# KRLGroup/gym-ma-survival-2d

Hardware: NVIDIA B200
Metric: agent_steps_per_sec (higher is better)
Workload: dtype f32

## Files before the change

### gym-ma-survival-2d_b200/csrc/msv_env.cuh

```cuda
#pragma once
#include "msv_device.cuh"
#include "msv_types.cuh"
#include "msv_launch.h"

enum { F_CX, F_CY, F_A, F_VX, F_VY, F_W, F_C0X, F_C0Y, F_A0, F_ALPHA0, F_SLEEP,
       F_FAT0, F_FAT1, F_FAT2, F_FAT3, F_FLAGS, F_QS, F_QC, F_COUNT };
enum { G_X, G_Y, G_HX, G_HY, G_AX, G_AY, G_ROT, G_F0, G_F1, G_F2, G_F3, G_COUNT };
enum { K_META, K_SEQ, K_MTYPE, K_LNX, K_LNY, K_LPX, K_LPY, K_NI, K_TI, K_NM, K_TM, K_COUNT };
enum { KS_NX = K_SEQ, KS_NY = K_MTYPE, KS_PX = K_LNX, KS_PY = K_LNY, KS_RBX = K_LPX, KS_RBY = K_LPY };

#define FL_ALIVE 1
#define FL_AWAKE 2
#define FL_ISLAND 4
#define FL_MOVED 8

#define KIND_NONE 0
#define KIND_AGENT 1
#define KIND_BOX 2
#define KIND_ITEM 3
#define KIND_HEAL 4
#define KIND_WALL 5

#define STREAM_SHUFFLE 0
#define STREAM_BOX 1
// ... 13 lines not shown
  int sid;
  int b;
  int flags;
  Manifold m;
  float ni, ti;
  f2 normal, rA, rB;
  float normalMass, tangentMass;
};

struct BodyS { f2 c; float a; f2 v; float w; float invM, invI; };

extern __shared__ float msv_sm[];


#ifndef MSV_INLINE_MASK
#define MSV_INLINE_MASK 0
#endif
#ifndef MSV_TOI_COOP
#define MSV_TOI_COOP 0
#endif
#ifndef MSV_FIXPOINT
#define MSV_FIXPOINT 1
#endif
#if (MSV_INLINE_MASK >> 0) & 1
#define COLD0 __device__ __forceinline__
#else
#define COLD0 __device__ __noinline__
#endif
#if (MSV_INLINE_MASK >> 1) & 1
#define COLD1 __device__ __forceinline__
#else
#define COLD1 __device__ __noinline__
#endif
#if (MSV_INLINE_MASK >> 2) & 1
#define COLD2 __device__ __forceinline__
#else
#define COLD2 __device__ __noinline__
#endif
#if (MSV_INLINE_MASK >> 3) & 1
#define COLD3 __device__ __forceinline__
#else
#define COLD3 __device__ __noinline__
#endif
#if (MSV_INLINE_MASK >> 4) & 1
#define COLD4 __device__ __forceinline__
#else
#define COLD4 __device__ __noinline__
#endif

__device__ __noinline__ double2 philox_uniform2_of(const DevConst& C, uint32_t genv, uint32_t episode, uint32_t step, uint32_t stream, uint32_t blk) {
  uint32_t o[4];
  philox4x32(genv, episode, step, (stream << 16) | blk, C.seed_lo, C.seed_hi, o);
  return make_double2(((double)(o[0] >> 5) * 67108864.0 + (double)(o[1] >> 6)) / 9007199254740992.0,
                      ((double)(o[2] >> 5) * 67108864.0 + (double)(o[3] >> 6)) / 9007199254740992.0);
}

__device__ __noinline__ void draw_reset(const DevConst& C, uint32_t genv, uint32_t episode, float* rec) {
  const int n = C.grid_n;
  unsigned char perm[64];
  for (int k = 0; k < n; ++k) perm[k] = (unsigned char)k;
  double2 up = make_double2(0.0, 0.0);
  for (int i = n - 1; i >= 1; --i) {
    const uint32_t kd = (uint32_t)(n - 1 - i);
    if (!(kd & 1u)) up = philox_uniform2_of(C, genv, episode, 0u, STREAM_SHUFFLE, kd >> 1);
    const double u = (kd & 1u) ? up.y : up.x;
    const int j = (int)(u * (i + 1));
    const unsigned char t = perm[i]; perm[i] = perm[j]; perm[j] = t;
  }
  int top = n;
  for (int b = 0; b < C.B0; ++b) {
    float hx = C.box_h, hy = C.box_h;
    if (C.box_randomized) {
// ... 72 lines not shown
  DEV void gsync() const { __syncwarp(gmask); }
  template <class V> DEV V bc(V v) const { return __shfl_sync(gmask, v, 0, G); }
  template <class V> DEV V from(V v, int j) const { return __shfl_sync(gmask, v, j, G); }
  DEV unsigned or32(unsigned v) const {
#pragma unroll
    for (int o = 1; o < G; o <<= 1) v |= __shfl_xor_sync(gmask, v, o, G);
    return v;
  }
  DEV unsigned long long or64(unsigned long long v) const {
#pragma unroll
    for (int o = 1; o < G; o <<= 1) v |= __shfl_xor_sync(gmask, v, o, G);
    return v;
  }
  DEV void share_counts() { int c = bc(nb | (ni << 8) | (nh << 16)); nb = c & 255; ni = (c >> 8) & 255; nh = (c >> 16) & 255; }
  DEV void share_bits() {
#pragma unroll
    for (int w = 0; w < PW; ++w) { ex[w] = bc(ex[w]); tc[w] = bc(tc[w]); en[w] = bc(en[w]); }
  }
  DEV void merge_bits() {
#pragma unroll
    for (int w = 0; w < PW; ++w) { ex[w] = or64(ex[w] & own[w]); tc[w] = or64(tc[w] & own[w]); en[w] = or64(en[w] & own[w]); }
  }

  DEV void take(const Env& o) {
    nb = o.nb; ni = o.ni; nh = o.nh; ntc = o.ntc;
#pragma unroll
    for (int w = 0; w < PW; ++w) { ex[w] = o.ex[w]; tc[w] = o.tc[w]; en[w] = o.en[w]; }
  }
#define MSV_COLD(call) do { Env c_(*this); c_.call; take(c_); } while (0)
#ifndef MSV_INLINE_MASK
#define MSV_INLINE_MASK 0
#endif
#define MSV_COLDK(k, call) do { if ((MSV_INLINE_MASK >> (k)) & 1) { call; } else { Env c_(*this); c_.call; take(c_); } } while (0)

  DEV float& AG(int f, int i) { return msv_sm[sb + (CHK_IDX(f, F_COUNT) * AC + CHK_IDX(i, AC))]; }
  DEV int& AGF(int i) { return reinterpret_cast<int*>(msv_sm)[sb + (F_FLAGS * AC + CHK_IDX(i, AC))]; }
  DEV float& BX(int f, int k) { return msv_sm[sb + (W_BOX + CHK_IDX(f, G_COUNT) * BC + CHK_IDX(k, BC))]; }
  DEV int& BXROT(int k) { return reinterpret_cast<int*>(msv_sm)[sb + (W_BOX + G_ROT * BC + CHK_IDX(k, BC))]; }
  DEV float& KF(int f, int k) { return msv_sm[sb + (W_TC + CHK_IDX(f, K_COUNT) * MAXC + CHK_IDX(k, MAXC))]; }
  DEV int& KI(int f, int k) { return reinterpret_cast<int*>(msv_sm)[sb + (W_TC + CHK_IDX(f, K_COUNT) * MAXC + CHK_IDX(k, MAXC))]; }
  DEV int& NTC() { return reinterpret_cast<int*>(msv_sm)[sb + (W_MISC + 0)]; }
  DEV float& ITP(int c, int k) { return msv_sm[sb + (W_ITEM + CHK_IDX(c, 2) * BC + CHK_IDX(k, BC))]; }
  DEV float& HLP(int c, int k) { return msv_sm[sb + (W_HEAL + CHK_IDX(c, 2) * HC + CHK_IDX(k, HC))]; }
  DEV int& LI(int k) { return reinterpret_cast<int*>(msv_sm)[sb + (W_LEAD + CHK_IDX(k, L_COUNT))]; }
  DEV unsigned& LU(int k) { return reinterpret_cast<unsigned*>(msv_sm)[sb + (W_LEAD + CHK_IDX(k, L_COUNT))]; }
  DEV float& LF(int k) { return msv_sm[sb + (W_LEAD + CHK_IDX(k, L_COUNT))]; }
  DEV float& TOIA(int i, int k) { return msv_sm[sb + (W_TOI + CHK_IDX(i, AC) * (BC + 4) + CHK_IDX(k, BC + 4))]; }
  DEV int& OVF() { return reinterpret_cast<int*>(msv_sm)[sb + (W_MISC + 1)]; }
  DEV bool alive(int i) { return AGF(i) & FL_ALIVE; }
  DEV bool awake(int i) { return AGF(i) & FL_AWAKE; }
  DEV f2 apos(int i) { return mk2(AG(F_CX, i), AG(F_CY, i)); }
  DEV static int meta_pack(int p, int a, int sid, int b) { return p | ((a + 1) << 8) | ((sid < 0 ? 0 : sid) << 12) | (b << 16); }
  DEV static void meta_unpack(int m, int& p, int& a, int& sid, int& b) { p = m & 255; a = ((m >> 8) & 15) - 1; sid = (m >> 12) & 15; b = (m >> 16) & 15; }

  DEV static bool bit(const unsigned long long* m, int p) {
    unsigned long long w = m[0];
// ... 194 lines not shown
  }
  DEV void box_change_health(int k, int delta, int cz) {
    int4 b1 = S.box1[k * N + e];
    if (!(b1.y & 1)) return;
    if (b1.w != MSV_CAUSE_NONE && cz != b1.w) return;
    b1.x += delta; b1.z = cz;
    S.box1[k * N + e] = b1;
  }
  DEV int inv_n(int i) { return LI(L_INV + (i)) & 7; }
  DEV int inv_kind(int i, int s) { return (LI(L_INV + (i)) >> (4 + 2 * s)) & 3; }
  DEV void inv_push(int i, int kind, float4 payload) {
    int n = inv_n(i);
    LI(L_INV + (i)) = (LI(L_INV + (i)) & ~(3 << (4 + 2 * n)) & ~7) | (kind << (4 + 2 * n)) | (n + 1);
    if (kind == MSV_ITEM_BOX) S.ainv[(i * 4 + n) * N + e] = payload;
  }
  DEV int inv_pop(int i, float4& payload) {
    int n = inv_n(i) - 1;
    int kind = inv_kind(i, n);
    if (kind == MSV_ITEM_BOX) payload = S.ainv[(i * 4 + n) * N + e];
    LI(L_INV + (i)) = (LI(L_INV + (i)) & ~7) | n;
    return kind;
  }

  COLD3 void remove_box(int k) {
    for (int i = 0; i < C.A; ++i) {
      int p = p_ab(i, k);
      if (bit(ex, p) && bit(tc, p)) wake(i);
      for (int q = k; q + 1 < nb; ++q) {
        int pd = p_ab(i, q), ps = p_ab(i, q + 1);
        if (bit(ex, ps)) { setb(ex, pd); S.pseq[pd * N + e] = S.pseq[ps * N + e]; S.pimp[pd * N + e] = S.pimp[ps * N + e]; } else clrb(ex, pd);
        if (bit(tc, ps)) setb(tc, pd); else clrb(tc, pd);
        if (bit(en, ps)) setb(en, pd); else clrb(en, pd);
      }
      int pl = p_ab(i, nb - 1);
      clrb(ex, pl); clrb(tc, pl); clrb(en, pl);
    }
    for (int q = k; q + 1 < nb; ++q) {
      S.box0[q * N + e] = S.box0[(q + 1) * N + e];
      S.box1[q * N + e] = S.box1[(q + 1) * N + e];
      S.boxseq[q * N + e] = S.boxseq[(q + 1) * N + e];
      BX(G_X, q) = BX(G_X, q + 1); BX(G_Y, q) = BX(G_Y, q + 1); BX(G_HX, q) = BX(G_HX, q + 1);
      BX(G_HY, q) = BX(G_HY, q + 1); BX(G_AX, q) = BX(G_AX, q + 1); BX(G_AY, q) = BX(G_AY, q + 1);
      BXROT(q) = BXROT(q + 1);
      BX(G_F0, q) = BX(G_F0, q + 1); BX(G_F1, q) = BX(G_F1, q + 1); BX(G_F2, q) = BX(G_F2, q + 1); BX(G_F3, q) = BX(G_F3, q + 1);
    }
    nb--;
  }
// ... 34 lines not shown
  DEV void candidates_of(int j, unsigned long long* cand, bool only_moved = false) {
    const int fj_ = AGF(j);
    if (!(fj_ & FL_ALIVE)) return;
    const bool mj = !only_moved || (fj_ & FL_MOVED);
    float fj[4]; agent_fat(j, fj);
    for (int i = 0; i < j; ++i) {
      const int fi_ = AGF(i);
      if (!(fi_ & FL_ALIVE)) continue;
      if (!mj && !(fi_ & FL_MOVED)) continue;
      int p = p_aa(i, j);
      if (bit(ex, p)) continue;
      float fi[4]; agent_fat(i, fi);
      if (aabb_overlap(fi, fj)) setb(cand, p);
    }
    if (!mj) return;
    for (int k = 0; k < BC + 4; ++k) {
      if (k < BC && k >= nb) continue;
      int p = k < BC ? p_ab(j, k) : p_aw(j, k - BC);
      if (bit(ex, p)) continue;
      float fs[4]; static_fat(k, fs);
      if (aabb_overlap(fj, fs)) setb(cand, p);
    }
  }
  COLD2 void number_candidates(unsigned long long* cand) {
    for (;;) {
      int best = -1; unsigned bestKey = 0xFFFFFFFFu;
      for (int w = 0; w < PW; ++w) {
        unsigned long long m = cand[w];
        while (m) {
          int p = w * 64 + __ffsll((long long)m) - 1; m &= m - 1;
          int a, sid, b; decode(p, a, sid, b);
          int s1 = a >= 0 ? agent_seq(a) : static_seq(sid), s2 = agent_seq(b);
          int lo = s1 < s2 ? s1 : s2, hi = s1 < s2 ? s2 : s1;
          unsigned key = ((unsigned)lo << 16) | (unsigned)hi;
          if (key < bestKey) { bestKey = key; best = p; }
        }
      }
      if (best < 0) break;
      clrb(cand, best);
      setb(ex, best); setb(en, best); clrb(tc, best);
      S.pseq[best * N + e] = (uint32_t)(++LI(L_CONTACTSEQ));
      S.pimp[best * N + e] = make_float2(0.0f, 0.0f);
    }
  }
  DEV void find_new_contacts(bool only_moved = false) {
    unsigned long long cand[PW];
#pragma unroll
    for (int w = 0; w < PW; ++w) cand[w] = 0ull;
    for (int j = g; j < C.A; j += G) candidates_of(j, cand, only_moved);
    bool any = false;
#pragma unroll
    for (int w = 0; w < PW; ++w) { cand[w] = or64(cand[w]); any |= cand[w] != 0ull; }
    if (any) {
      if (lead) {
        int nset = 0;
#pragma unroll
        for (int w = 0; w < PW; ++w) nset += __popcll(cand[w]);
        if (nset == 1) {
          int p = 0;
#pragma unroll
          for (int w = 0; w < PW; ++w) if (cand[w]) p = w * 64 + __ffsll((long long)cand[w]) - 1;
          setb(ex, p); setb(en, p); clrb(tc, p);
          S.pseq[p * N + e] = (uint32_t)(++LI(L_CONTACTSEQ));
          S.pimp[p * N + e] = make_float2(0.0f, 0.0f);
        } else { RARE_BEGIN(); unsigned long long cc[PW]; for (int w = 0; w < PW; ++w) cc[w] = cand[w]; MSV_COLDK(2, number_candidates(cc)); RARE_END(6); }
      }
      share_bits();
    }
  }
  DEV void find_new_contacts_of(int b) {
    unsigned long long cand[PW];
#pragma unroll
    for (int w = 0; w < PW; ++w) cand[w] = 0ull;
    candidates_of(b, cand);
    float fb[4]; agent_fat(b, fb);
    for (int j = b + 1; j < C.A; ++j) {
      if (!(AGF(j) & FL_ALIVE)) continue;
      const int p = p_aa(b, j);
      if (bit(ex, p)) continue;
      float fj[4]; agent_fat(j, fj);
      if (aabb_overlap(fb, fj)) setb(cand, p);
    }
    bool any = false;
#pragma unroll
    for (int w = 0; w < PW; ++w) any |= cand[w] != 0ull;
    if (any) number_candidates(cand);
  }

// ... 246 lines not shown
    float r = C.agent_r;
    float c0x = AG(F_C0X, i), c0y = AG(F_C0Y, i), cx = AG(F_CX, i), cy = AG(F_CY, i);
    float a1[4] = {c0x - r, c0y - r, c0x + r, c0y + r};
    float a2[4] = {cx - r, cy - r, cx + r, cy + r};
    float ab[4] = {fmin_(a1[0], a2[0]), fmin_(a1[1], a2[1]), fmax_(a1[2], a2[2]), fmax_(a1[3], a2[3])};
    float f0 = AG(F_FAT0, i), f1 = AG(F_FAT1, i), f2_ = AG(F_FAT2, i), f3 = AG(F_FAT3, i);
    if (f0 <= ab[0] && f1 <= ab[1] && ab[2] <= f2_ && ab[3] <= f3) return;
    float n0 = ab[0] - B2_AABB_EXT, n1 = ab[1] - B2_AABB_EXT, n2 = ab[2] + B2_AABB_EXT, n3 = ab[3] + B2_AABB_EXT;
    float dx = B2_AABB_MULT * (cx - c0x), dy = B2_AABB_MULT * (cy - c0y);
    if (dx < 0.0f) n0 += dx; else n2 += dx;
    if (dy < 0.0f) n1 += dy; else n3 += dy;
    AG(F_FAT0, i) = n0; AG(F_FAT1, i) = n1; AG(F_FAT2, i) = n2; AG(F_FAT3, i) = n3;
    AGF(i) |= FL_MOVED;
  }

  template <int NRr>
  DEV void island_single(int i, int cnt, unsigned long long ord, float h, float dtRatio) {
    f2 cB = apos(i);
    AG(F_C0X, i) = cB.x; AG(F_C0Y, i) = cB.y; AG(F_A0, i) = AG(F_A, i);
    f2 vB = mk2(C.damp * AG(F_VX, i), C.damp * AG(F_VY, i)); float wB = AG(F_W, i) * C.damp;
    f2 nrm[NRr], pp[NRr];
    bool ok = true;
    if (cnt > 0) {
      f2 rB[NRr]; float nm[NRr], tm[NRr], ni_[NRr], ti_[NRr]; int pr[NRr];
#pragma unroll (NRr <= NR ? NRr : 1)
      for (int k = 0; k < NRr; ++k) {
        if (k < cnt) {
          int s = (int)((ord >> (5 * k)) & 31ull);
          int a_, sid, b_; meta_unpack(KI(K_META, s), pr[k], a_, sid, b_);
          ni_[k] = dtRatio * KF(K_NI, s); ti_[k] = dtRatio * KF(K_TI, s);
          init_velocity_static(sid, mk2(KF(K_LNX, s), KF(K_LNY, s)), mk2(KF(K_LPX, s), KF(K_LPY, s)), cB,
                               nrm[k], pp[k], rB[k], nm[k], tm[k]);
        }
      }
#pragma unroll (NRr <= NR ? NRr : 1)
      for (int k = 0; k < NRr; ++k) if (k < cnt) warm_start_static(nrm[k], rB[k], ni_[k], ti_[k], vB, wB);
      for (int it = 0; it < 10; ++it) {
        const f2 v_in = vB; const float w_in = wB; bool changed = false;
#pragma unroll (NRr <= NR ? NRr : 1)
        for (int k = 0; k < NRr; ++k) if (k < cnt) {
          const float n0 = ni_[k], t0 = ti_[k];
          solve_velocity_static(nrm[k], rB[k], nm[k], tm[k], ni_[k], ti_[k], vB, wB);
          changed |= (__float_as_uint(ni_[k]) != __float_as_uint(n0)) | (__float_as_uint(ti_[k]) != __float_as_uint(t0));
        }
        if (MSV_FIXPOINT && !changed && __float_as_uint(vB.x) == __float_as_uint(v_in.x) && __float_as_uint(vB.y) == __float_as_uint(v_in.y) &&
            __float_as_uint(wB) == __float_as_uint(w_in)) break;
      }
#pragma unroll (NRr <= NR ? NRr : 1)
      for (int k = 0; k < NRr; ++k) if (k < cnt) S.pimp[pr[k] * N + e] = make_float2(ni_[k], ti_[k]);
    }
    AG(F_VX, i) = vB.x; AG(F_VY, i) = vB.y; AG(F_W, i) = wB;
    integrate_position(i, h);
    if (cnt > 0) {
      ok = false;
      cB = apos(i);
      for (int it = 0; it < 10 && !ok; ++it) {
        float minSep = 0.0f;
#pragma unroll (NRr <= NR ? NRr : 1)
        for (int k = 0; k < NRr; ++k) if (k < cnt) minSep = fmin_(minSep, solve_position_static(nrm[k], pp[k], cB, false));
        ok = minSep >= -3.0f * B2_LINEAR_SLOP;
      }
      AG(F_CX, i) = cB.x; AG(F_CY, i) = cB.y;
    }
    {
      const float linTol = B2_LIN_SLEEP_TOL * B2_LIN_SLEEP_TOL, angTol = B2_ANG_SLEEP_TOL * B2_ANG_SLEEP_TOL;
      float w = AG(F_W, i); f2 v = mk2(AG(F_VX, i), AG(F_VY, i));
      float st;
      if (w * w > angTol || vdot(v, v) > linTol) st = 0.0f; else st = AG(F_SLEEP, i) + h;
      AG(F_SLEEP, i) = st;
      if (ok && st >= B2_TIME_TO_SLEEP) sleep_body(i);
    }
    synchronize_fixtures(i);
  }
  DEV void solve_single(int i, float h, float dtRatio) {
    int f = AGF(i);
    if (!(f & FL_ALIVE) || !(f & FL_AWAKE)) return;
    AGF(i) = f | FL_ISLAND;
    unsigned long long ord = 0ull; int cnt = 0; unsigned taken = 0;
    for (;;) {
      int best = -1, bestSeq = -1;
      for (int k = 0; k < ntc; ++k) {
        if ((taken >> k) & 1u) continue;
        int p, a_, sid, b_; meta_unpack(KI(K_META, k), p, a_, sid, b_);
        if (b_ != i || a_ >= 0) continue;
        if (!bit(en, p) || !bit(tc, p)) continue;
        int sq = KI(K_SEQ, k);
        if (sq > bestSeq) { bestSeq = sq; best = k; }
      }
      if (best < 0) break;
      taken |= 1u << best;
      ord |= (unsigned long long)best << (5 * cnt); cnt++;
    }
    SUB_BEGIN();
    if (cnt <= NR) island_single<NR>(i, cnt, ord, h, dtRatio);
    else island_single<BC + 4>(i, cnt, ord, h, dtRatio);
    SUBMAX(cnt <= NR ? 6 : 7, cnt);
  }

  struct Ord { unsigned long long lo, hi; };
  DEV static int ord_get(const Ord& o, int k) { return k < 12 ? (int)((o.lo >> (5 * k)) & 31ull) : (int)((o.hi >> (5 * (k - 12))) & 31ull); }
  DEV static void ord_put(Ord& o, int k, int v) { if (k < 12) o.lo |= (unsigned long long)v << (5 * k); else o.hi |= (unsigned long long)v << (5 * (k - 12)); }
  static constexpr int NP = 3;
  DEV void island_pair(unsigned inisl, int nc, const Ord& ord, float h, float dtRatio) {
    const int X = __ffs((int)inisl) - 1, Y = 31 - __clz((int)inisl);
    f2 cX = apos(X), cY = apos(Y);
    f2 vX = mk2(AG(F_VX, X), AG(F_VY, X)), vY = mk2(AG(F_VX, Y), AG(F_VY, Y));
    float wX = AG(F_W, X), wY = AG(F_W, Y), aX = AG(F_A, X), aY = AG(F_A, Y);
    const float mI = C.inv_mass, iI = C.inv_I;
    int ty[NP], pr[NP];
    f2 nrm[NP], px[NP], rB[NP]; float nm[NP], tm[NP], ni_[NP], ti_[NP];
#pragma unroll
    for (int k = 0; k < NP; ++k) {
      ty[k] = 0; pr[k] = 0; nrm[k] = mk2(0.f, 0.f); px[k] = nrm[k]; rB[k] = nrm[k]; nm[k] = tm[k] = ni_[k] = ti_[k] = 0.0f;
      if (k >= nc) continue;
      const int s = ord_get(ord, k);
      int a_, sid, b_; meta_unpack(KI(K_META, s), pr[k], a_, sid, b_);
      ni_[k] = dtRatio * KF(K_NI, s); ti_[k] = dtRatio * KF(K_TI, s);
      if (a_ >= 0) {
// ... 92 lines not shown
          cY = vadd(cY, vmul(mI, Pv)); aY += iI * vcross(rB_, Pv);
        }
        minSep = fmin_(minSep, separation);
      }
      ok = minSep >= -3.0f * B2_LINEAR_SLOP;
    }
    AG(F_CX, X) = cX.x; AG(F_CY, X) = cX.y; AG(F_A, X) = aX; AG(F_CX, Y) = cY.x; AG(F_CY, Y) = cY.y; AG(F_A, Y) = aY;
    {
      const float linTol = B2_LIN_SLEEP_TOL * B2_LIN_SLEEP_TOL, angTol = B2_ANG_SLEEP_TOL * B2_ANG_SLEEP_TOL;
      bool can_sleep = ok;
#pragma unroll
      for (int q = 0; q < 2; ++q) {
        const int i = q == 0 ? X : Y;
        float w = AG(F_W, i); f2 v = mk2(AG(F_VX, i), AG(F_VY, i));
        float st;
        if (w * w > angTol || vdot(v, v) > linTol) st = 0.0f; else st = AG(F_SLEEP, i) + h;
        AG(F_SLEEP, i) = st;
        if (!(st >= B2_TIME_TO_SLEEP)) can_sleep = false;
      }
      if (can_sleep) { sleep_body(X); sleep_body(Y); }
    }
    synchronize_fixtures(X); synchronize_fixtures(Y);
  }
  COLD0 void solve_island(int seed, float h, float dtRatio) {
    SUB_BEGIN();
    Ord ord; ord.lo = 0ull; ord.hi = 0ull;
    int nc = 0; unsigned taken = 0, inisl = 1u << seed;
    {
      unsigned stack = (unsigned)seed; int sc = 1;
      AGF(seed) |= FL_ISLAND;
      while (sc > 0) {
        --sc;
        const int bI = (int)((stack >> (4 * sc)) & 15u);
        wake(bI);
        for (;;) {
          int best = -1, bestSeq = -1, bestMeta = 0;
          for (int k = 0; k < ntc; ++k) {
            if ((taken >> k) & 1u) continue;
            const int meta = KI(K_META, k);
            int p, a_, sid, b_; meta_unpack(meta, p, a_, sid, b_);
            if (a_ != bI && b_ != bI) continue;
            if (!bit(en, p) || !bit(tc, p)) continue;
            const int sq = KI(K_SEQ, k);
            if (sq > bestSeq) { bestSeq = sq; best = k; bestMeta = meta; }
          }
          if (best < 0) break;
          taken |= 1u << best;
// ... 192 lines not shown
    }
    gsync();
  }
  __device__ __forceinline__ void solve_find_new() {
    unsigned mv = 0;
    for (int i = g; i < C.A; i += G) if (AGF(i) & FL_MOVED) mv = 1u;
    if (or32(mv)) find_new_contacts(true);
  }

  DEV void advance(int i, float alpha) {
    float a0 = AG(F_ALPHA0, i);
    float beta = (alpha - a0) / (1.0f - a0);
    AG(F_C0X, i) += beta * (AG(F_CX, i) - AG(F_C0X, i));
    AG(F_C0Y, i) += beta * (AG(F_CY, i) - AG(F_C0Y, i));
    AG(F_A0, i) += beta * (AG(F_A, i) - AG(F_A0, i));
    AG(F_ALPHA0, i) = alpha;
    AG(F_CX, i) = AG(F_C0X, i); AG(F_CY, i) = AG(F_C0Y, i); AG(F_A, i) = AG(F_A0, i);
  }

  static constexpr int SNAPW = F_COUNT + 6 * PW + 1;
  static constexpr int TOI_ISL = 8;
  static_assert(SNAPW <= K_COUNT * (MAXC - TOI_ISL), "snapshot does not fit the scratch slots");
  DEV unsigned& SNAP(int q) { CHK((unsigned)q < (unsigned)SNAPW); return reinterpret_cast<unsigned*>(msv_sm)[sb + (W_TC + (q / (MAXC - TOI_ISL)) * MAXC + TOI_ISL + q % (MAXC - TOI_ISL))]; }
  COLD1 int toi_event(int minP, float minAlpha, float dt, int prevP) {
    SUB_BEGIN();
    int a, sid, b; decode(minP, a, sid, b);
    const float bk0 = AG(F_C0X, b), bk1 = AG(F_C0Y, b), bk2 = AG(F_CX, b), bk3 = AG(F_CY, b), bk4 = AG(F_A0, b), bk5 = AG(F_A, b), bk6 = AG(F_ALPHA0, b);
    advance(b, minAlpha);
    int nisl = 0;
    auto isl_add = [&](int sid_, const Manifold& m) {
      SBox bx = static_box(sid_);
      const f2 normal = qmul(bx.qs, bx.qc, m.localNormal), planePoint = sb_mul(bx, m.localPoint);
      KF(KS_NX, nisl) = normal.x; KF(KS_NY, nisl) = normal.y; KF(KS_PX, nisl) = planePoint.x; KF(KS_PY, nisl) = planePoint.y;
      nisl++;
    };
    {
      Manifold m_min; unsigned wk = 0;
      bool touching = contact_update(minP, a, sid, b, false, wk, &m_min);
      wake_all(wk);
      if (!touching) {
        clrb(en, minP);
        AG(F_C0X, b) = bk0; AG(F_C0Y, b) = bk1; AG(F_CX, b) = bk2; AG(F_CY, b) = bk3;
        AG(F_A0, b) = bk4; AG(F_A, b) = bk5; AG(F_ALPHA0, b) = bk6;
        return 0;
      }
      wake(b);
      isl_add(sid, m_min);
// ... 154 lines not shown
        gsync();
        cvalid |= need;
        while (need) {
          const int k = __ffs((int)need) - 1; need &= need - 1u;
          consider(k < BC ? p_ab(i, k) : p_aw(i, k - BC), TOIA(i, k));
        }
      }
#pragma unroll
      for (int o = 1; o < G; o <<= 1) {
        float oa = __shfl_xor_sync(gmask, minAlpha, o, G);
        int op = __shfl_xor_sync(gmask, minP, o, G), os = __shfl_xor_sync(gmask, minSeq, o, G);
        if (op >= 0 && (oa < minAlpha || (oa == minAlpha && os > minSeq))) { minAlpha = oa; minP = op; minSeq = os; }
      }
      if (minP < 0 || 1.0f - 10.0f * B2_EPS < minAlpha) break;
      int ea, ek, eb; decode(minP, ea, ek, eb);
      const bool mine = eb == g;
      if (mine) cvalid &= ~(1u << ek);
      gsync();
      int r = 0;
      TOIPROF(long long tpe = clock64();)
      if (lead) {
        RARE_BEGIN();
        if ((MSV_INLINE_MASK >> 1) & 1) r = toi_event(minP, minAlpha, dt, prevP);
        else { Env c_(*this); r = c_.toi_event(minP, minAlpha, dt, prevP); take(c_); }
        if (r & 1) prevP = minP;
        RARE_END(1);
      }
      gsync();
      r = bc(r);
      TOIPROF(tp_ev += clock64() - tpe; if (r & 1) tp_ran++; else tp_not++; if (r & 2) tp_same++;)
      share_bits();
      if (mine) {
        const unsigned long long c4 = (evcnt >> (4 * ek)) & 15ull;
        if (c4 < 15ull) evcnt += 1ull << (4 * ek);
      }
      if (!(r & 1)) continue;
      if (mine) {
        if (r & 2) {
          const unsigned long long c4 = (evcnt >> (4 * ek)) & 15ull;
          if (c4 <= (unsigned long long)C.toi_max_count) evcnt = (evcnt & ~(15ull << (4 * ek))) | ((unsigned long long)(C.toi_max_count + 1) << (4 * ek));
        } else cvalid = 0u;
      }
    }
    gsync();
    TOIPROF(if (lead) { unsigned long long tot = (unsigned long long)(clock64() - tp0); unsigned long long old = atomicMax(&g_toi[0], tot);
      if (tot > old) { g_toi[1] = tp_it; g_toi[2] = tp_ran; g_toi[3] = tp_not; g_toi[4] = tp_same; g_toi[5] = (unsigned long long)tp_ev; g_toi[6] = tot - (unsigned long long)tp_ev; g_toi[7] = tp_calls; g_toi[8] = (unsigned long long)e; } })
  }
// ... 5 lines not shown
      if (real) {
        const uint8_t* a = actions + ((size_t)e * C.A + i) * 6;
        a0 = min((int)a[0], 2); a1 = min((int)a[1], 2); a2 = min((int)a[2], 2);
        flags |= (a[3] ? 1u : 0u) << i | (a[4] ? 1u : 0u) << (8 + i) | (a[5] ? 1u : 0u) << (16 + i);
      }
      if (!alive(i)) continue;
      float s, c; rot_set(AG(F_A, i), s, c);
      AG(F_QS, i) = s; AG(F_QC, i) = c;
      float par = C.imp_par[a0], nor = C.imp_nor[a1];
      float ix = c * par + (-s) * nor, iy = s * par + c * nor;
      wake(i);
      AG(F_VX, i) += C.inv_mass * ix; AG(F_VY, i) += C.inv_mass * iy;
      AG(F_W, i) += C.inv_I * C.imp_ang[a2];
    }
    return or32(flags);
  }
  DEV void pre_use_give(unsigned act) {
    LI(L_USEHEAL) = 0; LI(L_USEBOX) = 0; LI(L_NEWBOX) = 0;
    bool any = LI(L_NP) > 0;
#pragma unroll
    for (int i = 0; i < AC; ++i) if (i < C.A && (((act >> (8 + i)) | (act >> (16 + i))) & 1u) && (LI(L_INV + (i)) & 7) != 0 && alive(i)) any = true;
    if (any) { RARE_BEGIN(); MSV_COLDK(3, pre_use_give_body(act)); RARE_END(5); }
  }
  COLD3 void pre_use_give_body(unsigned act) {
    for (int q = 0; q < LI(L_NP); ++q) {
      float4 p0 = S.pend0[q * N + e];
      add_item(p0.x, p0.y, p0.z, p0.w, S.pend1[q * N + e]);
    }
    LI(L_NP) = 0;
#pragma unroll
    for (int i = 0; i < AC; ++i) {
      if (i >= C.A || !alive(i) || !((act >> (8 + i)) & 1u) || inv_n(i) == 0) continue;
      float4 pl; int kind = inv_pop(i, pl);
      if (kind == MSV_ITEM_HEAL) { LI(L_USEHEAL)++; agent_change_health(i, C.healing, MSV_CAUSE_NONE); }
      else {
        LI(L_USEBOX)++;
        if (nb >= BC) { LI(L_OVERFLOW)++; continue; }
        float L = C.box_item_offset;
        float qs = AG(F_QS, i), qc = AG(F_QC, i);
        f2 off = mk2(qc * L + (-qs) * 0.0f, qs * L + qc * 0.0f);
        float x = AG(F_CX, i) + off.x, y = AG(F_CY, i) + off.y;
        int reh = __float_as_int(pl.w) & 1;
        const float4 nb0 = make_float4(x, y, pl.x, pl.y);
        const int4 nb1 = make_int4(0, reh << 1, MSV_CAUSE_NONE, C.box_ownership ? __float_as_int(pl.z) : MSV_CAUSE_NONE);
        S.box0[nb * N + e] = nb0; S.box1[nb * N + e] = nb1;
        S.boxseq[nb * N + e] = LI(L_BODYSEQ)++;
        put_box(nb, nb0, nb1);
// ... 53 lines not shown
        }
#pragma unroll
        for (int j = 0; j < G; ++j) res[s * G + j] = from(r, j);
      }
      if (lead) {
#pragma unroll
        for (int i = 0; i < AC; ++i) {
          if (!((raymask >> i) & 1u)) continue;
          int kind = res[i] & 255, tidx = (res[i] >> 8) & 255;
          if (kind == KIND_NONE) continue;
          int cz = C.teams ? MSV_CAUSE_TEAM0 + team_of(i) : i;
          if (kind == KIND_AGENT) agent_change_health(tidx, -C.melee_damage, cz);
          else if (kind == KIND_BOX) box_change_health(tidx, -C.melee_damage, cz);
          if (C.melee_cooldown >= 0) LI(L_COOLDOWN + (i)) = C.melee_cooldown;
        }
      }
    }
    if (lead && C.melee_cooldown >= 0) {
#pragma unroll
      for (int i = 0; i < AC; ++i) if (LI(L_COOLDOWN + (i)) > 0) LI(L_COOLDOWN + (i))--;
    }
  }

  __device__ __noinline__ double philox_uniform(uint32_t step, uint32_t stream, uint32_t k) {
    uint32_t o[4];
    philox4x32(C.env_offset + (uint32_t)e, (uint32_t)LI(L_EPISODE), step, (stream << 16) | (k >> 1), C.seed_lo, C.seed_hi, o);
    uint32_t a = o[(k & 1) * 2], b = o[(k & 1) * 2 + 1];
    return ((double)(a >> 5) * 67108864.0 + (double)(b >> 6)) / 9007199254740992.0;
  }

  DEV bool in_cone(f2 pl) {
    bool inside = true;
#pragma unroll
    for (int v = 0; v < 4; ++v) {
      float d = vdot(mk2(C.cone_n[v][0], C.cone_n[v][1]), vsub(pl, mk2(C.cone_v[v][0], C.cone_v[v][1])));
      if (d > 0.0f) inside = false;
    }
    return inside;
  }
  DEV f2 target_pos(int t) {
    if (t < AC) return apos(t);
    t -= AC;
    if (t < BC) return mk2(BX(G_X, t), BX(G_Y, t));
    t -= BC;
    if (t < BC) return mk2(ITP(0, t), ITP(1, t));
    t -= BC;
    return mk2(HLP(0, t), HLP(1, t));
// ... 63 lines not shown

  __device__ __forceinline__ void post_step_boxes() {
    int4 b1s[BC];
#pragma unroll
    for (int j = 0; j < BC; ++j) if (j < nb) b1s[j] = S.box1[j * N + e];
    const int nb0 = nb; int removed = 0;
#pragma unroll
    for (int j = 0; j < BC; ++j) {
      if (j >= nb0) continue;
      const int k = j - removed;
      int4 b1 = b1s[j];
      if (!(b1.y & 1)) { b1.y |= 1; b1.x = C.box_health; S.box1[k * N + e] = b1; }
      if (b1.x <= 0) {
        if (LI(L_NP) < BC) {
          S.pend0[LI(L_NP) * N + e] = make_float4(BX(G_X, k), BX(G_Y, k), BX(G_HX, k), BX(G_HY, k));
          S.pend1[LI(L_NP) * N + e] = C.box_ownership ? b1.z : MSV_CAUSE_NONE;
          LI(L_NP)++;
        } else LI(L_OVERFLOW)++;
        { RARE_BEGIN(); MSV_COLDK(3, remove_box(k)); RARE_END(7); }
        removed++;
      }
    }
  }
  COLD3 void handle_deaths() {
    int total = 0;
    for (int i = 0; i < C.A; ++i) if ((LU(L_DMASK) >> i) & 1u) total += inv_n(i);
    int top = total;
    for (int i = 0; i < C.A; ++i) {
      if (!((LU(L_DMASK) >> i) & 1u)) continue;
      f2 me = apos(i);
      int n = inv_n(i);
      for (int j = 0; j < n; ++j) {
        double ang = 2 * 3.141592653589793 * philox_uniform((uint32_t)LI(L_STEPS), STREAM_DEATH, (uint32_t)(--top));
        f2 off = from_polar(C.drop_radius, (float)ang);
        float x = me.x + off.x, y = me.y + off.y;
        int kind = inv_kind(i, j);
        if (kind == MSV_ITEM_HEAL) add_heal(x, y);
        else { float4 pl = S.ainv[(i * 4 + j) * N + e]; add_item(x, y, pl.x, pl.y, __float_as_int(pl.z)); }
      }
      LI(L_INV + (i)) = 0;
    }
    for (int i = 0; i < C.A; ++i) if ((LU(L_DMASK) >> i) & 1u) LI(L_KCAUSE + (LI(L_NKILLS)++)) = LI(L_CAUSE + (i));
    for (int i = 0; i < C.A; ++i) if ((LU(L_DMASK) >> i) & 1u) kill_agent(i);
  }
  DEV static constexpr unsigned long long pairs_of(int i, int w) {
    unsigned long long m = 0ull;
    for (int j = 0; j < AC; ++j) if (j != i) { const int p = i < j ? j * (j - 1) / 2 + i : i * (i - 1) / 2 + j; if ((p >> 6) == w) m |= 1ull << (p & 63); }
    for (int k = 0; k < BC + 4; ++k) { const int p = k < BC ? NAA + i * BC + k : NAA + AC * BC + i * 4 + (k - BC); if ((p >> 6) == w) m |= 1ull << (p & 63); }
    return m;
  }
  DEV void kill_agents_empty(unsigned dm) {
#pragma unroll
    for (int i = 0; i < AC; ++i) if ((dm >> i) & 1u) LI(L_KCAUSE + (LI(L_NKILLS)++)) = LI(L_CAUSE + (i));
#pragma unroll
    for (int i = 0; i < AC; ++i) {
      if (!((dm >> i) & 1u)) continue;
#pragma unroll
      for (int j = 0; j < AC; ++j) {
        if (j == i) continue;
        const int p = i < j ? j * (j - 1) / 2 + i : i * (i - 1) / 2 + j;
        if (((ex[0] & tc[0]) >> p) & 1ull) wake(j);
      }
#pragma unroll
      for (int w = 0; w < PW; ++w) { const unsigned long long m = ~pairs_of(i, w); ex[w] &= m; tc[w] &= m; en[w] &= m; }
      AGF(i) = 0;
    }
  }
  COLD3 void pickup_agent(int i) {
    const float r2 = C.pickup_r * C.pickup_r;
    f2 me = apos(i);
    int lastSeq = -1;
    for (;;) {
      int bestSeq = 0x7FFFFFFF, bkind = KIND_NONE, bidx = -1;
      for (int k = 0; k < ni; ++k) {
        float4 it = S.item0[k * N + e]; f2 d = vsub(mk2(it.x, it.y), me);
        if (!(vdot(d, d) <= r2)) continue;
        int sq = S.item1[k * N + e].y;
        if (sq > lastSeq && sq < bestSeq) { bestSeq = sq; bkind = KIND_ITEM; bidx = k; }
      }
      for (int k = 0; k < nh; ++k) {
        float2 h = S.heal[k * N + e]; f2 d = vsub(mk2(h.x, h.y), me);
        if (!(vdot(d, d) <= r2)) continue;
        int sq = S.healseq[k * N + e];
        if (sq > lastSeq && sq < bestSeq) { bestSeq = sq; bkind = KIND_HEAL; bidx = k; }
      }
      if (bkind == KIND_NONE) break;
      lastSeq = bestSeq;
      if (inv_n(i) + 1 > C.inv_slots) continue;
      if (bkind == KIND_HEAL) { inv_push(i, MSV_ITEM_HEAL, make_float4(0.f, 0.f, 0.f, 0.f)); remove_heal(bidx); seen_remove(0, 16, bidx); }
      else {
        float4 it = S.item0[bidx * N + e]; int2 i1 = S.item1[bidx * N + e];
// ... 150 lines not shown
      for (int i = 0; i < AC; ++i) if (i == split) rs = rew[i];
      LF(L_SREW + (1)) += rs;
    }
#pragma unroll
    for (int i = 0; i < AC; ++i) if (i < (C.teams ? 2 : A)) LI(L_SKILLS + (i)) += lk[i];
    LI(L_STSTEPS) += 1; LI(L_STHEALS) += LI(L_USEHEAL); LI(L_STBOXES) += LI(L_USEBOX);
#pragma unroll
    for (int i = 0; i < AC; ++i) if (i < A) { O.rewards[(size_t)e * A + i] = rew[i]; LF(L_EPRET + (i)) += rew[i]; }
    O.dones[e] = done ? 1 : 0;
    if (done) {
#pragma unroll
      for (int i = 0; i < AC; ++i) if (i < A) O.episode_return[(size_t)e * A + i] = LF(L_EPRET + (i));
      O.episode_length[e] = LI(L_STEPS);
    }
    if (C.battle_royale) {
      int na = 0;
      for (int i = 0; i < A; ++i) na += alive(i);
      O.br_over[e] = na <= 1 ? 1 : 0;
      for (int i = 0; i < A; ++i) O.br_results[(size_t)e * A + i] = (na <= 1 && alive(i)) ? 1 : 0;
    }
    return done;
  }

  COLD4 void reset() {
    LI(L_EPISODE) += 1; LI(L_STEPS) = 0;
    float* rec = &msv_sm[sb + W_TC];
    static_assert(K_COUNT * MAXC >= MSV_SPARE_W, "scratch too small for a reset record");
    if (S.spare_ep[e] == LI(L_EPISODE)) {
      const float4* src = reinterpret_cast<const float4*>(S.spare + (size_t)e * MSV_SPARE_W);
      float4 v[MSV_SPARE_W / 4];
#pragma unroll
      for (int q = 0; q < MSV_SPARE_W / 4; ++q) v[q] = src[q];
#pragma unroll
      for (int q = 0; q < MSV_SPARE_W / 4; ++q) { rec[4 * q] = v[q].x; rec[4 * q + 1] = v[q].y; rec[4 * q + 2] = v[q].z; rec[4 * q + 3] = v[q].w; }
    } else draw_reset(C, C.env_offset + (uint32_t)e, (uint32_t)LI(L_EPISODE), rec);
    LI(L_BODYSEQ) = 0; LI(L_CONTACTSEQ) = 0; LI(L_FIRST) = 1; LI(L_NEWFIX) = 1;
    nb = 0; ni = 0; nh = 0; LI(L_NP) = 0;
#pragma unroll
    for (int w = 0; w < PW; ++w) { ex[w] = 0ull; tc[w] = 0ull; en[w] = 0ull; }
#pragma unroll 1
    for (int b = 0; b < C.B0; ++b) {
      const float4 nb0 = make_float4(rec[MSV_SP_BOX + 4 * b], rec[MSV_SP_BOX + 4 * b + 1], rec[MSV_SP_BOX + 4 * b + 2], rec[MSV_SP_BOX + 4 * b + 3]);
      const int4 nb1 = make_int4(C.box_health, 1, MSV_CAUSE_NONE, MSV_CAUSE_NONE);
      S.box0[b * N + e] = nb0; S.box1[b * N + e] = nb1;
      S.boxseq[b * N + e] = LI(L_BODYSEQ)++;
      put_box(b, nb0, nb1);
      nb++;
// ... 37 lines not shown
```

### gym-ma-survival-2d_b200/csrc/msv_kernels.cu

```cuda
#include <cstdlib>
#include "msv_env.cuh"
#include "msv_launch.h"

__device__ unsigned long long g_prof[64];
#ifdef MSV_PROFILE
#define MSV_BLK_MAX 2048
#define MSV_BLK_STAMPS 24
#define MSV_TR_MAX 4096
#define MSV_TR_ROWS 6
__device__ unsigned long long g_tr[2 * MSV_TR_ROWS * MSV_TR_MAX];
__device__ __forceinline__ unsigned long long gtime_ns() { unsigned long long t; asm volatile("mov.u64 %0, %%globaltimer;" : "=l"(t)); return t; }
#define TRACE(row, idx) do { if (threadIdx.x == 0 && (idx) < MSV_TR_MAX) g_tr[((C.tq_ticket & 1u) * MSV_TR_ROWS + (row)) * MSV_TR_MAX + (idx)] = gtime_ns(); } while (0)
__device__ unsigned long long g_blk[MSV_BLK_MAX * MSV_BLK_STAMPS];
#define BLK_STAMP() do { if (C.profile && threadIdx.x == 0 && blockIdx.x < MSV_BLK_MAX && blk_n < MSV_BLK_STAMPS) { g_blk[blockIdx.x * MSV_BLK_STAMPS + blk_n] = (unsigned long long)clock64(); blk_n++; } } while (0)
#define PROF(k) do { if (C.profile) { long long _t = clock64(); ph[k] += (unsigned long long)(_t - t_last); t_last = _t; } } while (0)
#define PROFW(k) do { if (C.profile) { long long _t = clock64(); wt[k] += (unsigned long long)(_t - t_last); t_last = _t; } } while (0)
#else
#define PROF(k) do { } while (0)
#define PROFW(k) do { } while (0)
#define BLK_STAMP() do { } while (0)
#define TRACE(row, idx) do { } while (0)
#endif

#define MSV_COLD_ON(env, call) do { if ((MSV_INLINE_MASK >> 4) & 1) { env.call; } else { auto c_ = env; c_.call; env.take(c_); } } while (0)
#ifndef MSV_SYNC_MASK_ALL
#define MSV_SYNC_MASK(G) ((G) >= 8 ? 0x3FF : 0x1F7)
#else
#define MSV_SYNC_MASK(G) (MSV_SYNC_MASK_ALL)
#endif
#ifdef MSV_NO_PHASE_SYNC
#define PHASE_SYNC(k) do { } while (0)
#else
#define PHASE_SYNC(k) do { if ((MSV_SYNC_MASK(G) >> (k)) & 1) __syncthreads(); PROFW(k); BLK_STAMP(); } while (0)
#endif
#define MSV_GROUP_SETUP(G)                                                                       \
  const int es = threadIdx.x / (G), g = threadIdx.x % (G);                                       \
  const int e = blockIdx.x * (blockDim.x / (G)) + es;   \
  const unsigned gmask = (((G) >= 32) ? 0xffffffffu : ((1u << (G)) - 1u)) << ((threadIdx.x & 31) & ~((G) - 1))

template <int AC, int BC, int HC, int G>
__global__ void __launch_bounds__(MSV_TPB)
k_step(const __grid_constant__ DevConst C, const __grid_constant__ DevState S,
       const __grid_constant__ DevOut Oc, const uint8_t* __restrict__ actions) {
  MSV_GROUP_SETUP(G);
  DevOut O = Oc;
  asm volatile("griddepcontrol.launch_dependents;" ::: "memory");
  if (C.pdl_wait) asm volatile("griddepcontrol.wait;" ::: "memory");
// ... 688 lines not shown
```

### profiles/make_table.py

```python
#!/usr/bin/env python
import json
import os
import re

ROOT = os.path.dirname(os.path.dirname(os.path.abspath(__file__)))
W = ['2v2', '1v1_heal_only', 'ffa', 'ffa_lidar']


def load(w):
    return json.loads(open(os.path.join(ROOT, 'profiles', f'bench_r02_{w}.json')).read().strip().splitlines()[-1])


def main():
    out = ['<!-- MEASURED_TABLE begin (profiles/make_table.py) -->',
           '| workload (`bench.py --workload`) | envs/GPU | ms/step | agent-steps/s (device) | `e2e` (rewards+dones) | `concurrent_groups` device / e2e | `e2e_obs` sync / pipelined | k_step / k_obs2 / k_lidar ms | k_step GB/s (frac of 6 534) | C port, 16 threads | GPU/CPU |',
           '|---|---|---|---|---|---|---|---|---|---|---|']
    for w in W:
        d = load(w); r = d['roofline']; k = r['kernel_ms_all']
        cpu = d.get('cpu_baseline', {}).get('value')
        out.append(f"| {w} | {d['config']['envs_per_gpu']} | {d['ms_per_step']:.4f} | {d['value']:.3e} | {d['e2e']['value']:.3e} | {d['concurrent_groups']['value']:.3e} / {d['concurrent_groups']['e2e']['value']:.3e} | "
                   f"{d['e2e_obs']['value']:.3e} / {d['e2e_obs']['pipelined']['value']:.3e} | {k['k_step']:.4f} / {k['k_obs']:.4f} / {k['k_lidar']:.4f} | "
                   f"{r['achieved']:.0f} ({r['frac']:.4f}) | {cpu:.3e} | {d['value'] / cpu:.0f}x |" if cpu else '| %s | n/a |' % w)
    d = load('2v2')
    ph = d.get('ms_per_step_by_episode_phase') or {}
    if ph:
        out.append('')
        out.append('2v2 by episode phase (all envs reset together, then timed windows): ' + ', '.join(f'{k}: {v:.3f} ms' for k, v in ph.items()) + '.')
    rp = d.get('cpu_baseline_ref_python')
    if rp:
        out.append(f"Reference Python on the shim (`cpu_baseline_ref_python`, build container, {rp['cores']} cores): {rp['value']:.3e} agent-steps/s "
                   f"= {rp['env_steps_per_sec_per_core']:.0f} env-steps/s per core.")
    cp = os.path.join(ROOT, 'profiles', 'counters.json')
    if os.path.exists(cp):
        c = json.load(open(cp))
        for tag in ('2v2', 'ffa'):
            if tag in c:
                x = c[tag]
                out.append(f"ncu `{x['kernel'].split('(')[0]}` ({x['envs_per_launch']} envs): {x['warp_inst_per_launch'] / 1e6:.1f} M warp instructions, "
                           f"{x['active_lanes_per_inst']:.1f} active lanes, issue slots {x['issue_slots_busy_pct']:.1f} % busy, DRAM {x['dram_bytes_per_launch'] / 1e6:.1f} MB per launch.")
    out.append('<!-- MEASURED_TABLE end -->')
    p = os.path.join(ROOT, 'DESIGN.md')
    s = open(p).read()
    block = '\n'.join(out)
    if 'MEASURED_TABLE begin' in s:
        s = re.sub(r'<!-- MEASURED_TABLE begin.*?MEASURED_TABLE end -->', lambda m: block, s, flags=re.S)
    else:
        s = s.replace('MEASURED_TABLE', block, 1)
    open(p, 'w').write(s)
    print(block)

# ... 4 lines not shown
```

Measured before the change: 608.8 million.

## Route cold paths through a single noinline trampoline passing register state by value

Replaces the per-function __noinline__ COLDn markers and whole-Env copies with one templated noinline cold_call trampoline. It reconstructs an Env from its constants, passes only the register-resident counts and bitmasks in and out, and runs a lambda. The large island_single<BC+4> path is also moved behind this trampoline, and a per-contact index array is dropped in favour of re-reading it from shared memory. The goal is less local-memory spilling and fewer copies of the large Env object at call sites in the hot kernel. The cost is more template instantiations and larger code size.

```diff
diff --git a/gym-ma-survival-2d_b200/csrc/msv_env.cuh b/gym-ma-survival-2d_b200/csrc/msv_env.cuh
--- a/gym-ma-survival-2d_b200/csrc/msv_env.cuh
+++ b/gym-ma-survival-2d_b200/csrc/msv_env.cuh
@@ -59,32 +59,6 @@
 #ifndef MSV_FIXPOINT
 #define MSV_FIXPOINT 1
 #endif
-#if (MSV_INLINE_MASK >> 0) & 1
-#define COLD0 __device__ __forceinline__
-#else
-#define COLD0 __device__ __noinline__
-#endif
-#if (MSV_INLINE_MASK >> 1) & 1
-#define COLD1 __device__ __forceinline__
-#else
-#define COLD1 __device__ __noinline__
-#endif
-#if (MSV_INLINE_MASK >> 2) & 1
-#define COLD2 __device__ __forceinline__
-#else
-#define COLD2 __device__ __noinline__
-#endif
-#if (MSV_INLINE_MASK >> 3) & 1
-#define COLD3 __device__ __forceinline__
-#else
-#define COLD3 __device__ __noinline__
-#endif
-#if (MSV_INLINE_MASK >> 4) & 1
-#define COLD4 __device__ __forceinline__
-#else
-#define COLD4 __device__ __noinline__
-#endif
-
 __device__ __noinline__ double2 philox_uniform2_of(const DevConst& C, uint32_t genv, uint32_t episode, uint32_t step, uint32_t stream, uint32_t blk) {
   uint32_t o[4];
   philox4x32(genv, episode, step, (stream << 16) | blk, C.seed_lo, C.seed_hi, o);
@@ -203,16 +177,32 @@
     for (int w = 0; w < PW; ++w) { ex[w] = or64(ex[w] & own[w]); tc[w] = or64(tc[w] & own[w]); en[w] = or64(en[w] & own[w]); }
   }
 
-  DEV void take(const Env& o) {
+  struct Regs {
+    int nb, ni, nh, ntc, r;
+    unsigned long long ex[PW], tc[PW], en[PW];
+  };
+  DEV Regs regs() const {
+    Regs o; o.nb = nb; o.ni = ni; o.nh = nh; o.ntc = ntc; o.r = 0;
+#pragma unroll
+    for (int w = 0; w < PW; ++w) { o.ex[w] = ex[w]; o.tc[w] = tc[w]; o.en[w] = en[w]; }
+    return o;
+  }
+  DEV void take(const Regs& o) {
     nb = o.nb; ni = o.ni; nh = o.nh; ntc = o.ntc;
 #pragma unroll
     for (int w = 0; w < PW; ++w) { ex[w] = o.ex[w]; tc[w] = o.tc[w]; en[w] = o.en[w]; }
   }
-#define MSV_COLD(call) do { Env c_(*this); c_.call; take(c_); } while (0)
-#ifndef MSV_INLINE_MASK
-#define MSV_INLINE_MASK 0
-#endif
-#define MSV_COLDK(k, call) do { if ((MSV_INLINE_MASK >> (k)) & 1) { call; } else { Env c_(*this); c_.call; take(c_); } } while (0)
+  template <class Fn>
+  static __device__ __noinline__ Regs cold_call(const DevConst& C, const DevState& S, int es, int g, unsigned gmask, int e, Regs r, Fn fn) {
+    Env c(C, S, es, g, gmask, e);
+    c.take(r);
+    const int res = fn(c);
+    r = c.regs();
+    r.r = res;
+    return r;
+  }
+  template <class Fn> DEV int cold(Fn fn) { const Regs o = cold_call(C, S, es, g, gmask, e, regs(), fn); take(o); return o.r; }
+#define MSV_COLDK(k, call) do { if ((MSV_INLINE_MASK >> (k)) & 1) { call; } else { cold([=](Env& c_) mutable { c_.call; return 0; }); } } while (0)
 
   DEV float& AG(int f, int i) { return msv_sm[sb + (CHK_IDX(f, F_COUNT) * AC + CHK_IDX(i, AC))]; }
   DEV int& AGF(int i) { return reinterpret_cast<int*>(msv_sm)[sb + (F_FLAGS * AC + CHK_IDX(i, AC))]; }
@@ -453,7 +443,7 @@
     return kind;
   }
 
-  COLD3 void remove_box(int k) {
+  DEV void remove_box(int k) {
     for (int i = 0; i < C.A; ++i) {
       int p = p_ab(i, k);
       if (bit(ex, p) && bit(tc, p)) wake(i);
@@ -534,7 +524,7 @@
       if (aabb_overlap(fj, fs)) setb(cand, p);
     }
   }
-  COLD2 void number_candidates(unsigned long long* cand) {
+  DEV void number_candidates(unsigned long long* cand) {
     for (;;) {
       int best = -1; unsigned bestKey = 0xFFFFFFFFu;
       for (int w = 0; w < PW; ++w) {
@@ -575,7 +565,7 @@
           setb(ex, p); setb(en, p); clrb(tc, p);
           S.pseq[p * N + e] = (uint32_t)(++LI(L_CONTACTSEQ));
           S.pimp[p * N + e] = make_float2(0.0f, 0.0f);
-        } else { RARE_BEGIN(); unsigned long long cc[PW]; for (int w = 0; w < PW; ++w) cc[w] = cand[w]; MSV_COLDK(2, number_candidates(cc)); RARE_END(6); }
+        } else { RARE_BEGIN(); MSV_COLDK(2, number_candidates(cand)); RARE_END(6); }
       }
       share_bits();
     }
@@ -868,12 +858,12 @@
     f2 nrm[NRr], pp[NRr];
     bool ok = true;
     if (cnt > 0) {
-      f2 rB[NRr]; float nm[NRr], tm[NRr], ni_[NRr], ti_[NRr]; int pr[NRr];
+      f2 rB[NRr]; float nm[NRr], tm[NRr], ni_[NRr], ti_[NRr];
 #pragma unroll (NRr <= NR ? NRr : 1)
       for (int k = 0; k < NRr; ++k) {
         if (k < cnt) {
           int s = (int)((ord >> (5 * k)) & 31ull);
-          int a_, sid, b_; meta_unpack(KI(K_META, s), pr[k], a_, sid, b_);
+          int p_, a_, sid, b_; meta_unpack(KI(K_META, s), p_, a_, sid, b_);
           ni_[k] = dtRatio * KF(K_NI, s); ti_[k] = dtRatio * KF(K_TI, s);
           init_velocity_static(sid, mk2(KF(K_LNX, s), KF(K_LNY, s)), mk2(KF(K_LPX, s), KF(K_LPY, s)), cB,
                                nrm[k], pp[k], rB[k], nm[k], tm[k]);
@@ -893,7 +883,10 @@
             __float_as_uint(wB) == __float_as_uint(w_in)) break;
       }
 #pragma unroll (NRr <= NR ? NRr : 1)
-      for (int k = 0; k < NRr; ++k) if (k < cnt) S.pimp[pr[k] * N + e] = make_float2(ni_[k], ti_[k]);
+      for (int k = 0; k < NRr; ++k) if (k < cnt) {
+        const int pk = KI(K_META, (int)((ord >> (5 * k)) & 31ull)) & 255;
+        S.pimp[pk * N + e] = make_float2(ni_[k], ti_[k]);
+      }
     }
     AG(F_VX, i) = vB.x; AG(F_VY, i) = vB.y; AG(F_W, i) = wB;
     integrate_position(i, h);
@@ -939,7 +932,7 @@
     }
     SUB_BEGIN();
     if (cnt <= NR) island_single<NR>(i, cnt, ord, h, dtRatio);
-    else island_single<BC + 4>(i, cnt, ord, h, dtRatio);
+    else cold([=](Env& c_) { c_.template island_single<BC + 4>(i, cnt, ord, h, dtRatio); return 0; });
     SUBMAX(cnt <= NR ? 6 : 7, cnt);
   }
 
@@ -1078,7 +1071,7 @@
     }
     synchronize_fixtures(X); synchronize_fixtures(Y);
   }
-  COLD0 void solve_island(int seed, float h, float dtRatio) {
+  DEV void solve_island(int seed, float h, float dtRatio) {
     SUB_BEGIN();
     Ord ord; ord.lo = 0ull; ord.hi = 0ull;
     int nc = 0; unsigned taken = 0, inisl = 1u << seed;
@@ -1317,7 +1310,7 @@
   static constexpr int TOI_ISL = 8;
   static_assert(SNAPW <= K_COUNT * (MAXC - TOI_ISL), "snapshot does not fit the scratch slots");
   DEV unsigned& SNAP(int q) { CHK((unsigned)q < (unsigned)SNAPW); return reinterpret_cast<unsigned*>(msv_sm)[sb + (W_TC + (q / (MAXC - TOI_ISL)) * MAXC + TOI_ISL + q % (MAXC - TOI_ISL))]; }
-  COLD1 int toi_event(int minP, float minAlpha, float dt, int prevP) {
+  DEV int toi_event(int minP, float minAlpha, float dt, int prevP) {
     SUB_BEGIN();
     int a, sid, b; decode(minP, a, sid, b);
     const float bk0 = AG(F_C0X, b), bk1 = AG(F_C0Y, b), bk2 = AG(F_CX, b), bk3 = AG(F_CY, b), bk4 = AG(F_A0, b), bk5 = AG(F_A, b), bk6 = AG(F_ALPHA0, b);
@@ -1518,7 +1511,7 @@
       if (lead) {
         RARE_BEGIN();
         if ((MSV_INLINE_MASK >> 1) & 1) r = toi_event(minP, minAlpha, dt, prevP);
-        else { Env c_(*this); r = c_.toi_event(minP, minAlpha, dt, prevP); take(c_); }
+        else r = cold([=](Env& c_) { return c_.toi_event(minP, minAlpha, dt, prevP); });
         if (r & 1) prevP = minP;
         RARE_END(1);
       }
@@ -1570,7 +1563,7 @@
     for (int i = 0; i < AC; ++i) if (i < C.A && (((act >> (8 + i)) | (act >> (16 + i))) & 1u) && (LI(L_INV + (i)) & 7) != 0 && alive(i)) any = true;
     if (any) { RARE_BEGIN(); MSV_COLDK(3, pre_use_give_body(act)); RARE_END(5); }
   }
-  COLD3 void pre_use_give_body(unsigned act) {
+  DEV void pre_use_give_body(unsigned act) {
     for (int q = 0; q < LI(L_NP); ++q) {
       float4 p0 = S.pend0[q * N + e];
       add_item(p0.x, p0.y, p0.z, p0.w, S.pend1[q * N + e]);
@@ -1670,7 +1663,7 @@
     }
   }
 
-  __device__ __noinline__ double philox_uniform(uint32_t step, uint32_t stream, uint32_t k) {
+  DEV double philox_uniform(uint32_t step, uint32_t stream, uint32_t k) {
     uint32_t o[4];
     philox4x32(C.env_offset + (uint32_t)e, (uint32_t)LI(L_EPISODE), step, (stream << 16) | (k >> 1), C.seed_lo, C.seed_hi, o);
     uint32_t a = o[(k & 1) * 2], b = o[(k & 1) * 2 + 1];
@@ -1780,7 +1773,7 @@
       }
     }
   }
-  COLD3 void handle_deaths() {
+  DEV void handle_deaths() {
     int total = 0;
     for (int i = 0; i < C.A; ++i) if ((LU(L_DMASK) >> i) & 1u) total += inv_n(i);
     int top = total;
@@ -1824,7 +1817,7 @@
       AGF(i) = 0;
     }
   }
-  COLD3 void pickup_agent(int i) {
+  DEV void pickup_agent(int i) {
     const float r2 = C.pickup_r * C.pickup_r;
     f2 me = apos(i);
     int lastSeq = -1;
@@ -2021,7 +2014,7 @@
     return done;
   }
 
-  COLD4 void reset() {
+  DEV void reset() {
     LI(L_EPISODE) += 1; LI(L_STEPS) = 0;
     float* rec = &msv_sm[sb + W_TC];
     static_assert(K_COUNT * MAXC >= MSV_SPARE_W, "scratch too small for a reset record");
diff --git a/gym-ma-survival-2d_b200/csrc/msv_kernels.cu b/gym-ma-survival-2d_b200/csrc/msv_kernels.cu
--- a/gym-ma-survival-2d_b200/csrc/msv_kernels.cu
+++ b/gym-ma-survival-2d_b200/csrc/msv_kernels.cu
@@ -22,7 +22,7 @@
 #define TRACE(row, idx) do { } while (0)
 #endif
 
-#define MSV_COLD_ON(env, call) do { if ((MSV_INLINE_MASK >> 4) & 1) { env.call; } else { auto c_ = env; c_.call; env.take(c_); } } while (0)
+#define MSV_COLD_ON(env, call) do { if ((MSV_INLINE_MASK >> 4) & 1) { env.call; } else { env.cold([=](decltype(env)& c_) { c_.call; return 0; }); } } while (0)
 #ifndef MSV_SYNC_MASK_ALL
 #define MSV_SYNC_MASK(G) ((G) >= 8 ? 0x3FF : 0x1F7)
 #else
diff --git a/profiles/make_table.py b/profiles/make_table.py
--- a/profiles/make_table.py
+++ b/profiles/make_table.py
@@ -7,8 +7,18 @@
 W = ['2v2', '1v1_heal_only', 'ffa', 'ffa_lidar']
 
 
+def load_r02(w):
+    return json.loads(open(os.path.join(ROOT, 'profiles', f'bench_r02_{w}.json')).read().strip().splitlines()[-1])
+
+
 def load(w):
-    return json.loads(open(os.path.join(ROOT, 'profiles', f'bench_r02_{w}.json')).read().strip().splitlines()[-1])
+    p = os.path.join(ROOT, 'profiles', f'bench_r03_{w}.jsonl')
+    if not os.path.exists(p):
+        return load_r02(w)
+    runs = sorted((json.loads(x) for x in open(p).read().strip().splitlines()), key=lambda d: d['ms_per_step'])
+    d = runs[len(runs) // 2]
+    d['cpu_baseline'] = load_r02(w).get('cpu_baseline')
+    return d
 
 
 def main():
@@ -21,11 +31,11 @@
         out.append(f"| {w} | {d['config']['envs_per_gpu']} | {d['ms_per_step']:.4f} | {d['value']:.3e} | {d['e2e']['value']:.3e} | {d['concurrent_groups']['value']:.3e} / {d['concurrent_groups']['e2e']['value']:.3e} | "
                    f"{d['e2e_obs']['value']:.3e} / {d['e2e_obs']['pipelined']['value']:.3e} | {k['k_step']:.4f} / {k['k_obs']:.4f} / {k['k_lidar']:.4f} | "
                    f"{r['achieved']:.0f} ({r['frac']:.4f}) | {cpu:.3e} | {d['value'] / cpu:.0f}x |" if cpu else '| %s | n/a |' % w)
-    d = load('2v2')
+    d = load_r02('2v2')
     ph = d.get('ms_per_step_by_episode_phase') or {}
     if ph:
         out.append('')
-        out.append('2v2 by episode phase (all envs reset together, then timed windows): ' + ', '.join(f'{k}: {v:.3f} ms' for k, v in ph.items()) + '.')
+        out.append('2v2 by episode phase, round-2 build (all envs reset together, then timed windows): ' + ', '.join(f'{k}: {v:.3f} ms' for k, v in ph.items()) + '.')
     rp = d.get('cpu_baseline_ref_python')
     if rp:
         out.append(f"Reference Python on the shim (`cpu_baseline_ref_python`, build container, {rp['cores']} cores): {rp['value']:.3e} agent-steps/s "
diff --git a/profiles/sass_counts.py b/profiles/sass_counts.py
--- /dev/null
+++ b/profiles/sass_counts.py
@@ -0,0 +1,14 @@
+import re
+import sys
+
+ins = []
+for line in open(sys.argv[1]):
+    m = re.match(r'\s*/\*([0-9a-f]{4,})\*/\s+(.*?);', line)
+    if m: ins.append((int(m.group(1), 16), m.group(2)))
+targets = sorted({int(t, 16) for _, s in ins for t in re.findall(r'CALL\.\S+\s+(?:\S+\s+)?(0x[0-9a-f]+)', s)})
+end = min(targets) if targets else 1 << 62
+body = [s for a, s in ins if a < end]
+def cnt(lst, op): return sum(1 for s in lst if re.search(r'(^|\s)' + op + r'(\.|\s)', s))
+print(f"total {len(ins)} instructions; body (before the first callee, at {end:#x}) {len(body)}; {len(targets)} distinct call targets")
+for op in ("LDL", "STL", "CALL"):
+    print(f"  {op}: body {cnt(body, op)}, whole {cnt([s for _, s in ins], op)}")
```

Result: faster. 640.3 million, median of 6 (+5.2%).
